# furiosa-ai/eta-inversion

Hardware: AMD Instinct MI355X
Metric: images/sec SD1.5 512^2 50-step etainv+ptp (higher is better)
Workload: dtype bf16; 1 GPU; etainv+ptp, SD1.5-shaped UNet (seeded synthetic weights), 512x512 (64x64 latents), 50 DDIM steps, 32 image pairs per GPU per step, eta [[0.6, 0], [1, 0.7]], n=10 noise candidates, cfg 7.5/1; images_per_gpu=32, unet_sample_forwards_per_image_reference=300

## Files before the change

### eta-inversion_amd/csrc/attention.hip

```cpp
#include <cstdlib>
#include <type_traits>

#include "common.h"
#include "kernels.h"
#include "self_attn_route.h"

namespace etainv {

template <typename T> struct Frag;
template <> struct Frag<f16> {
  typedef f16x8 v8;
  typedef f16x4 v4;
  static __device__ __forceinline__ f32x4 mfma(v8 a, v8 b, f32x4 c) { return __builtin_amdgcn_mfma_f32_16x16x32_f16(a, b, c, 0, 0, 0); }
};
template <> struct Frag<bf16> {
  typedef bf16x8 v8;
  typedef bf16x4 v4;
  static __device__ __forceinline__ f32x4 mfma(v8 a, v8 b, f32x4 c) { return __builtin_amdgcn_mfma_f32_16x16x32_bf16(a, b, c, 0, 0, 0); }
};

constexpr float NEG_BIG = -1.0e30f;

__device__ __forceinline__ void row_roles(int b, int n_img, int& half, int& role, int& img) {
  half = b / (2 * n_img);
// ... 657 lines not shown
        for (int qb = 0; qb < QB; ++qb) {
          v8 pf[4];
#pragma unroll
          for (int ks = 0; ks < 4; ++ks)
#pragma unroll
            for (int e = 0; e < 8; ++e) pf[ks][e] = (T)__builtin_amdgcn_exp2f(s[qb][ks >> 1][(ks & 1) * 8 + e]);
#pragma unroll
          for (int ks = 0; ks < 4; ++ks)
#pragma unroll
            for (int dt = 0; dt < DT; ++dt) o[qb][dt] = Frag32<T>::mfma(vf[ks][dt], pf[ks], o[qb][dt]);
        }
        if (j + 1 < ntiles) store_p(0, cur ^ 1);
        __syncthreads();
      }
    }

    const int q_base = qblk * QI + wid * (32 * QB);
#pragma unroll
    for (int qb = 0; qb < QB; ++qb) {
      const float l = __shfl(o[qb][GEO::LT][GEO::LI], r + 32 * GEO::LH, 64);
      const float inv = 1.f / l;
      const int query = q_base + qb * 32 + r;
      T* op = out + ((int64_t)b * N + query) * C + hd * D + 4 * h;
#pragma unroll
      for (int g4 = 0; g4 < D / 8; ++g4) {
        const int dt = g4 >> 2, i0 = (g4 & 3) * 4;
        T v[4] = {(T)(o[qb][dt][i0] * inv), (T)(o[qb][dt][i0 + 1] * inv), (T)(o[qb][dt][i0 + 2] * inv), (T)(o[qb][dt][i0 + 3] * inv)};
        *reinterpret_cast<u32x2*>(op + 8 * g4) = *reinterpret_cast<u32x2*>(v);
      }
    }
  }
}

template <typename T, int D, int QT, bool EDIT>
__global__ void __launch_bounds__(256) cross_attn_kernel(const T* __restrict__ q, const T* __restrict__ kv, T* __restrict__ out,
                                                         CrossParams p, int row0) {
  typedef typename Frag<T>::v8 v8;
  typedef typename Frag<T>::v4 v4;
  constexpr int DP = (D + 31) / 32 * 32;
  constexpr int KS = DP / 32;
  constexpr int DT = (D + 15) / 16;
  constexpr int NCH = D / 8;
  constexpr int KC = 96;
  constexpr int KT = 5;
  constexpr int KSTR = DP + 8;
  constexpr int VSTR = KC + 8;
  constexpr int PSTR = 81;

  extern __shared__ __attribute__((aligned(16))) char smem[];
  T* sK = reinterpret_cast<T*>(smem);
  T* sKs = sK + KC * KSTR;
  T* sVt = EDIT ? sKs + KC * KSTR : sKs;
  float* sP = reinterpret_cast<float*>(sVt + DT * 16 * VSTR);
  float* sTab = sP + 4 * QT * 16 * PSTR;

  const int tid = threadIdx.x, lane = tid & 63, wid = tid >> 6;
  const int fr = lane & 15, q4 = lane >> 4;
  int bx = blockIdx.x, gxn = gridDim.x, h = blockIdx.y, bz = blockIdx.z;
  if (p.xcd_gx > 0) {
    const int lin = blockIdx.x, xcd = lin & 7, t = lin >> 3;
    h = t % p.heads;
    const int c = (t / p.heads) * 8 + xcd;
    gxn = p.xcd_gx;
    bx = c % gxn;
    bz = c / gxn;
  }
// ... 18 lines not shown
  const bool do_edit = EDIT && p.edit && p.layout == 2 && is_cond && role == 1;
  const bool do_store = p.map_layer >= 0 && is_cond;
  const int bs = b - p.n_img;

  for (int idx = tid; idx < KC * (KSTR / 8); idx += 256) {
    const int key = idx / (KSTR / 8), ch = idx % (KSTR / 8);
    u32x4 a = {0u, 0u, 0u, 0u}, s = {0u, 0u, 0u, 0u};
    if (key < p.n_ctx && ch < NCH) {
      a = *reinterpret_cast<const u32x4*>(kv + ((int64_t)b * p.n_ctx + key) * C2 + h * D + ch * 8);
      if (do_edit) s = *reinterpret_cast<const u32x4*>(kv + ((int64_t)bs * p.n_ctx + key) * C2 + h * D + ch * 8);
    }
    *reinterpret_cast<u32x4*>(sK + key * KSTR + ch * 8) = a;
    if (EDIT) *reinterpret_cast<u32x4*>(sKs + key * KSTR + ch * 8) = s;
  }
  for (int idx = tid; idx < KC * NCH; idx += 256) {
    const int key = idx % KC, ch = idx / KC;
    u32x4 c = {0u, 0u, 0u, 0u};
    if (key < p.n_ctx) c = *reinterpret_cast<const u32x4*>(kv + ((int64_t)b * p.n_ctx + key) * C2 + C + h * D + ch * 8);
    const T* e = reinterpret_cast<const T*>(&c);
#pragma unroll
    for (int j = 0; j < 8; ++j) sVt[(ch * 8 + j) * VSTR + key] = e[j];
  }
  if (EDIT && do_edit && tid < p.n_ctx) {
    int mp = p.mapper ? p.mapper[img * 77 + tid] : 0;
    if (mp < 0) mp += p.n_ctx;
    sTab[0 * 80 + tid] = __builtin_bit_cast(float, mp);
    sTab[1 * 80 + tid] = p.alphas ? p.alphas[img * 77 + tid] : 0.f;
    sTab[2 * 80 + tid] = p.equalizer ? p.equalizer[img * 77 + tid] : 1.f;
    sTab[3 * 80 + tid] = p.cross_alpha[img * 77 + tid];
  }
  __syncthreads();

  constexpr bool QPF = D <= 80;
  u32x4 qn[QPF ? QT : 1][QPF ? 2 : 1][QPF ? KS : 1];
  auto load_q = [&](int qb, int qt, int brow, u32x4 (&dst)[QPF ? KS : 1]) __attribute__((always_inline)) {
    int query = qb * (64 * QT) + wid * (16 * QT) + qt * 16 + fr;
    query = query < N ? query : N - 1;
    const T* qp = q + ((int64_t)brow * N + query) * C + h * D;
#pragma unroll
    for (int ks = 0; ks < KS; ++ks) {
      const int d0 = ks * 32 + q4 * 8;
      u32x4 v = {0u, 0u, 0u, 0u};
      if (d0 < D) v = *reinterpret_cast<const u32x4*>(qp + d0);
      dst[ks] = v;
    }
  };
  auto load_block = [&](int qb) __attribute__((always_inline)) {
    if constexpr (QPF) {
#pragma unroll
      for (int qt = 0; qt < QT; ++qt) {
        load_q(qb, qt, b, qn[qt][0]);
        if (do_edit) load_q(qb, qt, bs, qn[qt][1]);
      }
    }
  };
  if (bx * (64 * QT) < N) load_block(bx);
  for (int qb = bx; qb * (64 * QT) < N; qb += gxn) {
  u32x4 qc[QPF ? QT : 1][QPF ? 2 : 1][QPF ? KS : 1];
  if constexpr (QPF) {
#pragma unroll
    for (int qt = 0; qt < QT; ++qt)
#pragma unroll
      for (int e = 0; e < 2; ++e)
#pragma unroll
        for (int ks = 0; ks < KS; ++ks) qc[qt][e][ks] = qn[qt][e][ks];
    if ((qb + gxn) * (64 * QT) < N) load_block(qb + gxn);
  }
#pragma unroll
  for (int qt = 0; qt < QT; ++qt) {
    const int q_base = qb * (64 * QT) + wid * (16 * QT);
    int query = q_base + qt * 16 + fr;
    const bool q_ok = query < N;
    query = q_ok ? query : N - 1;
    float* sPw = sP + ((wid * QT + qt) * 16 + fr) * PSTR;

    auto probs = [&](int brow, const T* keys, f32x4 (&pr)[KT]) {
      const T* qp = q + ((int64_t)brow * N + query) * C + h * D;
      f32x4 s[KT];
#pragma unroll
      for (int kt = 0; kt < KT; ++kt) s[kt] = (f32x4){0.f, 0.f, 0.f, 0.f};
#pragma unroll
      for (int ks = 0; ks < KS; ++ks) {
        const int d0 = ks * 32 + q4 * 8;
        u32x4 v = {0u, 0u, 0u, 0u};
        if constexpr (QPF) v = qc[qt][brow == b ? 0 : 1][ks];
        else if (d0 < D) v = *reinterpret_cast<const u32x4*>(qp + d0);
        v8 qf = *reinterpret_cast<v8*>(&v);
#pragma unroll
        for (int kt = 0; kt < KT; ++kt) {
          v8 kf = *reinterpret_cast<const v8*>(keys + (kt * 16 + fr) * KSTR + ks * 32 + q4 * 8);
          s[kt] = Frag<T>::mfma(kf, qf, s[kt]);
        }
      }
      float mx = NEG_BIG;
#pragma unroll
      for (int kt = 0; kt < KT; ++kt)
#pragma unroll
        for (int r = 0; r < 4; ++r) {
          float v = s[kt][r] * p.scale_log2;
          if (kt * 16 + q4 * 4 + r >= p.n_ctx) v = NEG_BIG;
          s[kt][r] = v;
          mx = fmaxf(mx, v);
        }
      mx = fmaxf(mx, __shfl_xor(mx, 16, 64));
      mx = fmaxf(mx, __shfl_xor(mx, 32, 64));
      float rs = 0.f;
#pragma unroll
      for (int kt = 0; kt < KT; ++kt)
#pragma unroll
        for (int r = 0; r < 4; ++r) {
          float e = __builtin_amdgcn_exp2f(s[kt][r] - mx);
          s[kt][r] = e;
          rs += e;
        }
      rs += __shfl_xor(rs, 16, 64);
      rs += __shfl_xor(rs, 32, 64);
      const float inv = 1.f / rs;
#pragma unroll
      for (int kt = 0; kt < KT; ++kt) pr[kt] = s[kt] * inv;
    };

    f32x4 pr[KT];
    if (do_edit) {
      f32x4 ps[KT];
      probs(bs, sKs, ps);
#pragma unroll
      for (int kt = 0; kt < KT; ++kt)
#pragma unroll
        for (int r = 0; r < 4; ++r) sPw[kt * 16 + q4 * 4 + r] = ps[kt][r];
      __builtin_amdgcn_fence(__ATOMIC_RELEASE, "workgroup");
      __builtin_amdgcn_wave_barrier();
      probs(b, sK, pr);
#pragma unroll
      for (int kt = 0; kt < KT; ++kt)
#pragma unroll
        for (int r = 0; r < 4; ++r) {
          const int key = kt * 16 + q4 * 4 + r;
          if (key < p.n_ctx) {
            const float tg = pr[kt][r];
            float rep;
            if (p.replace_mat) {
              const float* mrow = p.replace_mat + (int64_t)img * 77 * 77 + key;
              rep = 0.f;
              for (int w = 0; w < p.n_ctx; ++w) rep += sPw[w] * mrow[w * 77];
            } else {
              const int mp = __builtin_bit_cast(int, sTab[0 * 80 + key]);
              const float a = sTab[1 * 80 + key];
              rep = sPw[mp] * a + tg * (1.f - a);
            }
            rep *= sTab[2 * 80 + key];
            const float ca = sTab[3 * 80 + key];
            pr[kt][r] = rep * ca + (1.f - ca) * tg;
          }
        }
    } else {
      probs(b, sK, pr);
    }

    if (do_store && q_ok) {
      float* mp = p.maps_acc + (((((int64_t)p.map_layer * p.n_img_cap + img) * 2 + role) * p.heads + h) * N + query) * 77;
#pragma unroll
      for (int kt = 0; kt < KT; ++kt)
#pragma unroll
        for (int r = 0; r < 4; ++r) {
          const int key = kt * 16 + q4 * 4 + r;
          if (key < p.n_ctx) mp[key] += pr[kt][r];
        }
    }

    v8 pf[3];
#pragma unroll
    for (int kt = 0; kt < 6; ++kt)
#pragma unroll
      for (int r = 0; r < 4; ++r) pf[kt >> 1][(kt & 1) * 4 + r] = (kt < KT) ? (T)pr[kt < KT ? kt : 0][r] : (T)0.f;
    f32x4 acc[DT];
#pragma unroll
    for (int dt = 0; dt < DT; ++dt) acc[dt] = (f32x4){0.f, 0.f, 0.f, 0.f};
#pragma unroll
    for (int ks = 0; ks < 3; ++ks)
#pragma unroll
      for (int dt = 0; dt < DT; ++dt) {
        const T* vp = sVt + (dt * 16 + fr) * VSTR + ks * 32 + q4 * 4;
        v4 lo = *reinterpret_cast<const v4*>(vp);
        v4 hi = *reinterpret_cast<const v4*>(vp + 16);
        v8 vf = __builtin_shufflevector(lo, hi, 0, 1, 2, 3, 4, 5, 6, 7);
        acc[dt] = Frag<T>::mfma(vf, pf[ks], acc[dt]);
      }
    if (q_ok) {
      T* op = out + ((int64_t)b * N + query) * C + h * D;
#pragma unroll
      for (int dt = 0; dt < DT; ++dt) {
        const int dc = dt * 16 + q4 * 4;
        if (dc < D) {
          T o[4] = {(T)acc[dt][0], (T)acc[dt][1], (T)acc[dt][2], (T)acc[dt][3]};
          *reinterpret_cast<u32x2*>(op + dc) = *reinterpret_cast<u32x2*>(o);
        }
      }
    }
  }
  }
}

template <typename T, int D, int QB, int OCC>
static int launch_self40(const void* qkv, void* out, int b, int n, int heads, int mode, int n_img, int q_prescaled, hipStream_t s, int first_row = 0, int head_major = 0) {
  const int hm_rows = head_major ? b : 0;
  const int nqb = cdiv(n, 128 * QB);
  const bool remap = ((b * heads) % 8) == 0;
  const float q_scale = q_prescaled ? 1.0f : (1.0f / sqrtf((float)D)) * 1.4426950408889634f;
  constexpr size_t lds = A32<D>::LDS;
  ProfScope prof(PROF_SELF_ATTN, 4.0 * (double)b * heads * (double)n * (double)n * D, s);
  if constexpr (lds > 64 * 1024) {
    allow_dynamic_lds<&self_attn40_kernel<T, D, true, QB, OCC>>(lds);
    allow_dynamic_lds<&self_attn40_kernel<T, D, false, QB, OCC>>(lds);
  }
  if (remap)
    hipLaunchKernelGGL((self_attn40_kernel<T, D, true, QB, OCC>), dim3(nqb * heads * b), dim3(256), lds, s, (const T*)qkv, (T*)out, n, heads, q_scale, mode, n_img, nqb, first_row, hm_rows);
  else
    hipLaunchKernelGGL((self_attn40_kernel<T, D, false, QB, OCC>), dim3(nqb, heads, b), dim3(256), lds, s, (const T*)qkv, (T*)out, n, heads, q_scale, mode, n_img, nqb, first_row, hm_rows);
  ETAINV_LAUNCH_CHECK();
  return 0;
}

template <typename T, int D, int QB, int NW>
static int launch_self40q(const void* qkv, void* out, int b, int n, int heads, int mode, int n_img, int q_prescaled, hipStream_t s, int first_row, int head_major, int n_cu) {
  const int hm_rows = head_major ? b : 0;
  const int nqb = n / (32 * QB * NW);
  const int n_items = nqb * heads * b;
  const int remap = ((b * heads) % 8) == 0;
  const float q_scale = q_prescaled ? 1.0f : (1.0f / sqrtf((float)D)) * 1.4426950408889634f;
  constexpr size_t lds = (size_t)(4 * (A32<D>::KBUF + A32<D>::VBUF) + A32<D>::VBUF) * 2;
  allow_dynamic_lds<&self_attn40q_kernel<T, D, QB, NW, false>>(lds);
// ... 21 lines not shown
  }
  return n_cu[dev];
}

int launch_self_attention_mode(const void* qkv, void* out, int b, int n, int heads, int d, int mode, int n_img, int dtype,
                               hipStream_t s, int q_prescaled, int first_row, int head_major) {
  ETAINV_CHECK((!head_major && !q_prescaled) || self_attn_prescaled_hm_ok(d, dtype), "head-major QKV planes / pre-scaled queries: head_dim 40 / 80 on the 16-bit kernels only");
  ETAINV_CHECK(qkv && out && b > 0 && n > 0, "bad arguments");
  ETAINV_CHECK(mode >= 0 && mode <= 3, "self-attention mode: 0 plain, 1 ptp self-replace, 2 masactrl, 3 plug-and-play");
  ETAINV_CHECK(mode != 3 || (n_img > 0 && first_row == 0 && b == 3 * n_img), "plug-and-play mode needs the 3*n_img layout [u_s, u_t, c_t] x n_img with first_row == 0");
  ETAINV_CHECK(mode == 0 || mode == 3 || (n_img > 0 && ((first_row >= 0 && b + first_row == 4 * n_img && (first_row == 0 || (first_row == n_img && mode == 1))) ||
                                                        (first_row < 0 && b == 3 * n_img && mode == 1))),
               "ptp / masactrl modes need the 4*n_img backward layout (ptp: optionally without its first n_img rows, or rows [u_t, c_t, c_s] with first_row < 0)");
  if (dtype == ETAINV_F32) return launch_self_attention_f32(qkv, out, b, n, heads, d, mode, n_img, s, first_row);
  ETAINV_CHECK(d == 40 || d == 80 || d == 160, "head_dim must be 40, 80 or 160");
  const int n_cu = device_cu_count();
  const SelfAttnRoute route = self_attn_route(b, n, heads, d, n_cu, env_flag("ETAINV_A40_PERSIST", true), env_flag("ETAINV_A80_PERSIST", true));
  ETAINV_DISPATCH_HALF(dtype, T, switch (route) {
    case SELF_D40_ONE_BLOCK_PER_WAVE: return launch_self40<T, 40, 1, 2>(qkv, out, b, n, heads, mode, n_img, q_prescaled, s, first_row, head_major);
    case SELF_D40_PERSISTENT: return launch_self40q<T, 40, 4, 4>(qkv, out, b, n, heads, mode, n_img, q_prescaled, s, first_row, head_major, n_cu);
    case SELF_D40_TWO_BLOCK: return launch_self40<T, 40, 2, 2>(qkv, out, b, n, heads, mode, n_img, q_prescaled, s, first_row, head_major);
    case SELF_D80_PERSISTENT: return launch_self40q<T, 80, 2, 4>(qkv, out, b, n, heads, mode, n_img, q_prescaled, s, first_row, head_major, n_cu);
    case SELF_D80: return launch_self40<T, 80, 1, 2>(qkv, out, b, n, heads, mode, n_img, q_prescaled, s, first_row, head_major);
    case SELF_D160: return launch_self40<T, 160, 1, 1>(qkv, out, b, n, heads, mode, n_img, q_prescaled, s, first_row, head_major);
  });
  return 0;
}

template <typename T, int D>
static int launch_cross_t(const void* q, const void* kv, void* out, int b, const CrossParams& p, hipStream_t s) {
  constexpr int QT = 2;
  constexpr int DP = (D + 31) / 32 * 32, DT = (D + 15) / 16;
  const size_t lds_edit = (size_t)(2 * 96 * (DP + 8) + DT * 16 * (96 + 8)) * sizeof(T) + (size_t)(4 * QT * 16 * 81 + 4 * 80) * sizeof(float);
  const size_t lds_plain = (size_t)(96 * (DP + 8) + DT * 16 * (96 + 8)) * sizeof(T);
  allow_dynamic_lds<&cross_attn_kernel<T, D, QT, true>>(lds_edit);
  allow_dynamic_lds<&cross_attn_kernel<T, D, QT, false>>(lds_plain);
  ProfScope prof(PROF_CROSS_ATTN, 4.0 * (double)b * p.heads * (double)p.N * (double)p.n_ctx * D, s);
  const int nqb = cdiv(p.N, 64 * QT);
  auto launch = [&](bool edit, int row0, int rows) {
    static const int target_env = getenv("ETAINV_CROSS_BLOCKS") ? std::max(64, atoi(getenv("ETAINV_CROSS_BLOCKS"))) : 0;
    const int target = target_env ? target_env : p.N >= 2048 ? (edit ? 2048 : 6144) : 1024;
    const int cap = target_env ? nqb : p.N <= 256 ? 1 : p.N <= 1024 ? 2 : p.N <= 4096 ? 8 : nqb;
    const int gx = std::max(1, std::min(std::min(nqb, cap), cdiv(target, rows * p.heads)));
    const bool xcd_heads = env_flag("ETAINV_CROSS_XCD", true);
    CrossParams pl = p;
    dim3 grid(gx, p.heads, rows);
    if (xcd_heads && (gx * rows) % 8 == 0) {
      pl.xcd_gx = gx;
      grid = dim3(gx * p.heads * rows);
    }
    if (edit)
      hipLaunchKernelGGL((cross_attn_kernel<T, D, QT, true>), grid, dim3(256), lds_edit, s, (const T*)q, (const T*)kv, (T*)out, pl, row0);
    else
      hipLaunchKernelGGL((cross_attn_kernel<T, D, QT, false>), grid, dim3(256), lds_plain, s, (const T*)q, (const T*)kv, (T*)out, pl, row0);
  };
  if (p.edit && p.layout == 2) {
    const int edit0 = 3 * p.n_img - p.first_row;
    launch(false, 0, edit0);
    launch(true, edit0, b - edit0);
  } else {
    launch(false, 0, b);
  }
  ETAINV_LAUNCH_CHECK();
  return 0;
}

int launch_cross_attention_p(const void* q, const void* kv, void* out, int b, int d, const CrossParams& p, int dtype, hipStream_t s) {
// ... 22 lines not shown
```

### eta-inversion_amd/csrc/ppgemm.hip

```cpp
#include <cstdio>
#include <cstdlib>
#include <type_traits>
#include <vector>

#include "common.h"
#include "kernels.h"

namespace etainv {

namespace {

template <typename T> struct PMfma;
template <> struct PMfma<f16> {
  typedef f16x8 frag;
  static __device__ __forceinline__ f32x4 run(frag a, frag b, f32x4 c) { return __builtin_amdgcn_mfma_f32_16x16x32_f16(a, b, c, 0, 0, 0); }
};
template <> struct PMfma<bf16> {
  typedef bf16x8 frag;
  static __device__ __forceinline__ f32x4 run(frag a, frag b, f32x4 c) { return __builtin_amdgcn_mfma_f32_16x16x32_bf16(a, b, c, 0, 0, 0); }
};

#define PP_VMCNT(n) __builtin_amdgcn_s_waitcnt(0x0F70 | ((n) & 15) | (((n) >> 4) << 14))
#define PP_LGKMCNT0() __builtin_amdgcn_s_waitcnt(0xC07F)
#define PP_DMA(BYTES_INSN, voff32, sbase, ldsaddr) \
  asm volatile("s_mov_b32 m0, %2\n\ts_nop 0\n\t" BYTES_INSN " %0, %1" : : "v"(voff32), "s"(sbase), "s"(__builtin_amdgcn_readfirstlane(ldsaddr)) : "memory")

constexpr int PBM = 256, PBK = 64;
constexpr int PMT = 4;

__device__ __forceinline__ float dualn_row_sum16(float x) {
  x += __builtin_bit_cast(float, __builtin_amdgcn_update_dpp(0, __builtin_bit_cast(int, x), 0xB1, 0xf, 0xf, true));
  x += __builtin_bit_cast(float, __builtin_amdgcn_update_dpp(0, __builtin_bit_cast(int, x), 0x4E, 0xf, 0xf, true));
  x += __builtin_bit_cast(float, __builtin_amdgcn_update_dpp(0, __builtin_bit_cast(int, x), 0x141, 0xf, 0xf, true));
  x += __builtin_bit_cast(float, __builtin_amdgcn_update_dpp(0, __builtin_bit_cast(int, x), 0x140, 0xf, 0xf, true));
  return x;
}

template <int HN> struct DualN {
  static constexpr int NT = HN / 32;
  static constexpr int WN = HN / 2;
  static constexpr int BN2 = 2 * HN;
  static constexpr int PASSES = BN2 / 64;
  static constexpr int A_BYTES = PBM * PBK * 2, B_BYTES = BN2 * PBK * 2, SLOT = A_BYTES + B_BYTES;
  static constexpr int OFF_BIAS = 2 * SLOT, OFF_S = OFF_BIAS + 2 * BN2 * 4, OFF_STAT = OFF_S + 2 * BN2 * 4, LDS = OFF_STAT + 2 * PBM * 2 * 4;
};

template <typename T, int HN, int EPI, bool RES, int STAT, bool A2 = false>
__global__ void __launch_bounds__(512, 2) pp_dualn_kernel(IGemmParams p) {
  typedef typename PMfma<T>::frag frag;
  typedef DualN<HN> D;
  constexpr int NT = D::NT, WN = D::WN, BN2 = D::BN2, PASSES = D::PASSES;
  constexpr bool LNC = EPI != 0;
  static_assert((HN == 160 && EPI <= 2) || (HN == 128 && EPI == 3), "instantiations");
  static_assert(!LNC || (!RES && !STAT), "a LayerNorm consumer has no residual and emits no statistics");
  extern __shared__ __attribute__((aligned(16))) char smem[];
  float* sBias = reinterpret_cast<float*>(smem + D::OFF_BIAS);
  float* sS = reinterpret_cast<float*>(smem + D::OFF_S);
  float* sStat = reinterpret_cast<float*>(smem + D::OFF_STAT);

  const int tid = threadIdx.x, lane = tid & 63;
  const int wid = __builtin_amdgcn_readfirstlane(tid >> 6);
  const int wm = wid >> 1, wn = wid & 1;
  const int fr = lane & 15, fq = lane >> 4;
  const bool late = wid >= 4;

  const int K1 = p.c1, K = A2 ? p.c1 + p.c2 : p.c1, N = p.N;
  const int nk = K / PBK, nk1 = K1 / PBK;
  const int tiles_n = N / BN2;
  const int total_tiles = (p.M / PBM) * tiles_n;
  const int G = gridDim.x;
  const int my_tiles = (total_tiles - (int)blockIdx.x + G - 1) / G;
  if (my_tiles <= 0) return;
  auto tile_origin = [&](int i, int& m0, int& n0) __attribute__((always_inline)) {
    int v = blockIdx.x + i * G;
    if ((total_tiles & 7) == 0) v = (v & 7) * (total_tiles >> 3) + (v >> 3);
    const int tm = v / tiles_n;
    m0 = tm * PBM;
    n0 = (v - tm * tiles_n) * BN2;
  };
  const int total_steps = my_tiles * nk;
  const bool no_dma = p.debug & 1, no_epi = p.debug & 2, no_store = p.debug & 8, no_gelu = p.debug & 16;
  const bool fake_store = p.debug & 64;
  const bool has_bias = p.bias != nullptr;

  const unsigned lrow = tid >> 3;
  unsigned voff[PASSES];
#pragma unroll
  for (int q = 0; q < PASSES; ++q) voff[q] = ((lrow + 64 * q) * (unsigned)K + (((tid & 7) ^ (lrow & 7)) << 3)) * 2u;
  unsigned voa1[A2 ? 4 : 1], voa2[A2 ? 4 : 1];
  if constexpr (A2) {
#pragma unroll
    for (int q = 0; q < 4; ++q) {
      voa1[q] = ((lrow + 64 * q) * (unsigned)K1 + (((tid & 7) ^ (lrow & 7)) << 3)) * 2u;
      voa2[q] = ((lrow + 64 * q) * (unsigned)p.c2 + (((tid & 7) ^ (lrow & 7)) << 3)) * 2u;
    }
  }
  const int wrow_b = wid * 8 * PBK * 2;
  const unsigned lds0 = (unsigned)(unsigned long long)(__attribute__((address_space(3))) char*)smem;
  const char* a_base = nullptr;
  const char* a_base2 = nullptr;
  const char* w_base = nullptr;
  int a_tile = 0, a_kt = 0, a_cnt = 0;
  int b_tile = 0, b_kt = 0, b_cnt = 0;
  auto set_a = [&](int tile) __attribute__((always_inline)) {
    int m0, n0;
    tile_origin(tile, m0, n0);
    a_base = reinterpret_cast<const char*>(p.a1) + (int64_t)m0 * K1 * 2;
    if constexpr (A2) a_base2 = reinterpret_cast<const char*>(p.a2) + (int64_t)m0 * p.c2 * 2;
  };
  auto set_b = [&](int tile) __attribute__((always_inline)) {
    int m0, n0;
    tile_origin(tile, m0, n0);
    w_base = reinterpret_cast<const char*>(p.w) + (int64_t)n0 * K * 2;
    if (wid < BN2 / 64) {
      const unsigned db = ((tile & 1) * BN2 + wid * 64) * 4;
      if (has_bias) PP_DMA("global_load_lds_dword", (unsigned)(lane * 4), reinterpret_cast<const char*>(p.bias + n0 + wid * 64), lds0 + D::OFF_BIAS + db);
      if constexpr (LNC) PP_DMA("global_load_lds_dword", (unsigned)(lane * 4), reinterpret_cast<const char*>(p.ln_s + n0 + wid * 64), lds0 + D::OFF_S + db);
    }
    if constexpr (LNC)
      PP_DMA("global_load_lds_dword", (unsigned)(lane * 4), reinterpret_cast<const char*>(p.ln_stat + (int64_t)m0 * 2 + wid * 64),
             lds0 + D::OFF_STAT + ((tile & 1) * 512 + wid * 64) * 4);
  };
  auto issue_a = [&]() __attribute__((always_inline)) {
    if (!no_dma) {
      const unsigned d = lds0 + (a_cnt & 1) * D::SLOT + wrow_b;
      if constexpr (A2) {
        const bool second = a_kt >= nk1;
        const char* g = second ? a_base2 + (a_kt - nk1) * (PBK * 2) : a_base + a_kt * (PBK * 2);
        const unsigned v0 = second ? voa2[0] : voa1[0], v1 = second ? voa2[1] : voa1[1], v2 = second ? voa2[2] : voa1[2], v3 = second ? voa2[3] : voa1[3];
        PP_DMA("global_load_lds_dwordx4", v0, g, d);
        PP_DMA("global_load_lds_dwordx4", v1, g, d + 1 * (64 * PBK * 2));
        PP_DMA("global_load_lds_dwordx4", v2, g, d + 2 * (64 * PBK * 2));
        PP_DMA("global_load_lds_dwordx4", v3, g, d + 3 * (64 * PBK * 2));
      } else {
      const char* g = a_base + a_kt * (PBK * 2);
      PP_DMA("global_load_lds_dwordx4", voff[0], g, d);
      PP_DMA("global_load_lds_dwordx4", voff[1], g, d + 1 * (64 * PBK * 2));
      PP_DMA("global_load_lds_dwordx4", voff[2], g, d + 2 * (64 * PBK * 2));
      PP_DMA("global_load_lds_dwordx4", voff[3], g, d + 3 * (64 * PBK * 2));
      }
    }
    ++a_cnt;
    if (++a_kt == nk) {
      a_kt = 0;
      if (++a_tile < my_tiles) set_a(a_tile);
    }
  };
  auto issue_b = [&](auto q0_tag, auto q1_tag) __attribute__((always_inline)) {
    constexpr int q0 = decltype(q0_tag)::value, q1 = decltype(q1_tag)::value;
    if (!no_dma) {
      const char* g = w_base + b_kt * (PBK * 2);
      const unsigned d = lds0 + (b_cnt & 1) * D::SLOT + D::A_BYTES + wrow_b;
#pragma unroll
      for (int q = q0; q < q1; ++q) PP_DMA("global_load_lds_dwordx4", voff[q], g, d + q * (64 * PBK * 2));
    }
    if constexpr (q1 == PASSES) {
      ++b_cnt;
      if (++b_kt == nk) {
        b_kt = 0;
        if (++b_tile < my_tiles) set_b(b_tile);
      }
    }
  };

  f32x4 acc0[PMT][NT], acc1[PMT][NT];
#pragma unroll
  for (int i = 0; i < PMT; ++i)
#pragma unroll
    for (int j = 0; j < NT; ++j) acc0[i][j] = acc1[i][j] = (f32x4){0.f, 0.f, 0.f, 0.f};
  u32x4 fa[PMT] = {}, fb[NT] = {};
  unsigned a_rd[2], b_rd[2];
#pragma unroll
  for (int kk = 0; kk < 2; ++kk) {
    a_rd[kk] = ((wm * 64 + fr) * PBK + (((kk * 4 + fq) ^ (fr & 7)) << 3)) * 2;
    b_rd[kk] = D::A_BYTES + ((wn * WN + fr) * PBK + (((kk * 4 + fq) ^ (fr & 7)) << 3)) * 2;
  }
  auto read_a = [&](int slot, auto kk_tag) __attribute__((always_inline)) {
    const char* ba = smem + slot * D::SLOT + a_rd[decltype(kk_tag)::value];
#pragma unroll
    for (int i = 0; i < PMT; ++i) fa[i] = *reinterpret_cast<const u32x4*>(ba + i * (16 * PBK * 2));
  };
  auto read_b = [&](int slot, auto kk_tag, auto nh_tag) __attribute__((always_inline)) {
    const char* bb = smem + slot * D::SLOT + b_rd[decltype(kk_tag)::value] + decltype(nh_tag)::value * (HN * PBK * 2);
#pragma unroll
    for (int j = 0; j < NT; ++j) fb[j] = *reinterpret_cast<const u32x4*>(bb + j * (16 * PBK * 2));
  };
  auto cluster = [&](auto nh_tag) __attribute__((always_inline)) {
    constexpr int NH = decltype(nh_tag)::value;
    __builtin_amdgcn_sched_barrier(0);
    __builtin_amdgcn_s_setprio(1);
#pragma unroll
    for (int i = 0; i < PMT; ++i)
#pragma unroll
      for (int j = 0; j < NT; ++j) {
        if constexpr (NH == 0) acc0[i][j] = PMfma<T>::run(__builtin_bit_cast(frag, fb[j]), __builtin_bit_cast(frag, fa[i]), acc0[i][j]);
        else acc1[i][j] = PMfma<T>::run(__builtin_bit_cast(frag, fb[j]), __builtin_bit_cast(frag, fa[i]), acc1[i][j]);
      }
    __builtin_amdgcn_s_setprio(0);
    __builtin_amdgcn_sched_barrier(0);
  };

  T* const out = reinterpret_cast<T*>(p.out);
  const T* const res = reinterpret_cast<const T*>(p.residual);
  auto store_blocks = [&](T* prow, auto& po, auto nb_tag, int hm_d, int hm_skip) __attribute__((always_inline)) {
    constexpr int NB = decltype(nb_tag)::value;
    if (no_store) return;
    auto at = [&](int col) __attribute__((always_inline)) { return prow + col + (col >= hm_d ? hm_skip : 0); };
    if (fake_store) {
#pragma unroll
      for (int k = 0; k + 1 < NB; k += 2) {
        const u32x4 v = {po[k][0], po[k][1], po[k + 1][0], po[k + 1][1]};
        *reinterpret_cast<u32x4*>(prow + (k >> 1) * 512) = v;
      }
      if constexpr (NB & 1) *reinterpret_cast<u32x2*>(prow + (NB >> 1) * 512) = po[NB - 1];
      return;
    }
// ... 167 lines not shown
          }
          float mu = sum * (1.0f / (float)(NT * 4)), m2 = 0.f;
#pragma unroll
          for (int j = 0; j < NT; ++j) {
            T o[4];
            *reinterpret_cast<u32x2*>(o) = po[j];
#pragma unroll
            for (int q = 0; q < 4; ++q) { const float d = to_f32(o[q]) - mu; m2 += d * d; }
          }
          {
            const float mo = __shfl_xor(mu, 16, 64), qo = __shfl_xor(m2, 16, 64);
            const bool odd = fq & 1;
            float ma = odd ? mo : mu, mb = odd ? mu : mo, qa = odd ? qo : m2, qb = odd ? m2 : qo;
            float d = mb - ma;
            ma += 0.5f * d;
            qa += qb + d * d * (0.5f * (float)(NT * 4));
            const float mo2 = __shfl_xor(ma, 32, 64), qo2 = __shfl_xor(qa, 32, 64);
            const bool hi = fq >> 1;
            float m_lo = hi ? mo2 : ma, m_hi = hi ? ma : mo2, q_lo = hi ? qo2 : qa, q_hi = hi ? qa : qo2;
            d = m_hi - m_lo;
            mu = m_lo + 0.5f * d;
            m2 = q_lo;
            m2 += q_hi + d * d * (0.5f * (float)(2 * NT * 4));
          }
          if (fq == 0) *reinterpret_cast<f32x2*>(p.stat_out + ((int64_t)(mrow + i * 16) * p.stat_P + n0 / 80 + wn) * 2) = (f32x2){mu, m2};
        }
      }
    }
  };

  typedef std::integral_constant<int, 0> I0;
  typedef std::integral_constant<int, 1> I1;
  constexpr int QA = 2, QB = PASSES == 5 ? 4 : 3;
  set_a(0);
  set_b(0);
  issue_a();
  issue_b(I0{}, std::integral_constant<int, PASSES>{});
  if (total_steps > 1) { issue_a(); PP_VMCNT(4); } else { PP_VMCNT(0); }
  __builtin_amdgcn_s_barrier();
  if (late) __builtin_amdgcn_s_barrier();

  int ct_kt = 0, ct_tile = 0;
  for (int s = 0; s < total_steps; ++s) {
    const int slot = s & 1;
    const bool next = s + 1 < total_steps;
    if (s > 0 && ct_kt == 0 && !no_epi) {
      epilogue_half(I0{}, ct_tile - 1);
      epilogue_half(I1{}, ct_tile - 1);
    }
    const bool issue_w = next;
    if (issue_w) issue_b(I0{}, std::integral_constant<int, QA>{});
    read_a(slot, I0{});
    read_b(slot, I0{}, I0{});
    PP_LGKMCNT0();
    __builtin_amdgcn_sched_barrier(0);
    __builtin_amdgcn_s_barrier();
    cluster(I0{});
    __builtin_amdgcn_s_barrier();
    if (issue_w) issue_b(std::integral_constant<int, QA>{}, std::integral_constant<int, QB>{});
    read_b(slot, I0{}, I1{});
    PP_LGKMCNT0();
    __builtin_amdgcn_sched_barrier(0);
    __builtin_amdgcn_s_barrier();
    cluster(I1{});
    __builtin_amdgcn_s_barrier();
    if (issue_w) issue_b(std::integral_constant<int, QB>{}, std::integral_constant<int, PASSES>{});
    read_a(slot, I1{});
    read_b(slot, I1{}, I0{});
    PP_LGKMCNT0();
    __builtin_amdgcn_sched_barrier(0);
    __builtin_amdgcn_s_barrier();
    cluster(I0{});
    __builtin_amdgcn_s_barrier();
    PP_VMCNT(0);
    if (s + 2 < total_steps) issue_a();
    read_b(slot, I1{}, I1{});
    PP_LGKMCNT0();
    __builtin_amdgcn_sched_barrier(0);
    __builtin_amdgcn_s_barrier();
    cluster(I1{});
    __builtin_amdgcn_s_barrier();
    if (++ct_kt == nk) { ct_kt = 0; ++ct_tile; }
  }
  if (!no_epi) {
    epilogue_half(I0{}, ct_tile - 1);
    epilogue_half(I1{}, ct_tile - 1);
  }
  if (!late) __builtin_amdgcn_s_barrier();
}

}

static int dualn_kind(const IGemmParams& p, int dtype) {
  if (!env_flag("ETAINV_DUALN", true) || (dtype != ETAINV_F16 && dtype != ETAINV_BF16)) return -1;
  if (p.taps != 1 || p.rowvec || p.out_f32 || p.out_nchw || p.w_batch_stride || p.ksplit > 1) return -1;
  if (p.a2 && (p.geglu || p.ln_stat || p.residual || p.stat_out || p.hm_heads || p.c2 % PBK != 0 || p.c2 <= 0 || !env_flag("ETAINV_DUALN_A2", true))) return -1;
  if (p.stat_out && p.rows_per_batch % 64 != 0) return -1;
  if (p.M % PBM != 0 || p.c1 % PBK != 0 || p.c1 < 2 * PBK) return -1;
  int kind;
  if (p.geglu) {
    if (!p.ln_stat || !p.ln_s || !p.bias || p.residual || p.stat_out || p.hm_heads || p.N % 256 != 0) return -1;
    kind = 3;
  } else if (p.ln_stat) {
    if (!p.ln_s || !p.bias || p.residual || p.stat_out || p.N % 320 != 0) return -1;
    kind = p.hm_heads ? 2 : 1;
    if (kind == 2 && ((p.hm_dim != 40 && p.hm_dim != 80) || p.hm_heads != 8 || p.N != 3 * 8 * p.hm_dim || p.hm_tokens % 256 != 0 || p.M % p.hm_tokens != 0)) return -1;
  } else {
    if (p.hm_heads || p.N % 320 != 0) return -1;
    kind = 0;
  }
  static const int min_tiles = env_int("ETAINV_DUALN_MIN_TILES", 192);
  const int64_t tiles = (int64_t)(p.M / PBM) * (p.N / (kind == 3 ? 256 : 320));
  const int64_t rounds = (tiles + 255) / 256;
  if (tiles < min_tiles || tiles * 5 < rounds * 256 * 4) return -1;
  return kind;
}
bool pp_dualn_applicable(const IGemmParams& p, int dtype) { return dualn_kind(p, dtype) >= 0; }
bool pp_dualn_hm_ok(const IGemmParams& p, int dtype) { return dualn_kind(p, dtype) == 2; }

template <typename T, int HN, int EPI, bool RES, int STAT, bool A2 = false>
static void launch_dualn_t(const IGemmParams& p, int grid, hipStream_t s) {
  allow_dynamic_lds<&pp_dualn_kernel<T, HN, EPI, RES, STAT, A2>>(DualN<HN>::LDS);
  hipLaunchKernelGGL((pp_dualn_kernel<T, HN, EPI, RES, STAT, A2>), dim3(grid), dim3(512), DualN<HN>::LDS, s, p);
}

int launch_pp_dualn(const IGemmParams& p_in, int dtype, hipStream_t s, int* stat_P) {
  IGemmParams p = p_in;
  const int kind = dualn_kind(p, dtype);
  ETAINV_CHECK(kind >= 0, "not a dual-N launch (ask pp_dualn_applicable first)");
  if (p.stat_out) p.stat_P = p.stat_kind == 1 ? 64 : p.N / 80;
  if (stat_P) *stat_P = p.stat_out ? p.stat_P : 0;
  IGemmPlan& plan = igemm_last_plan();
  plan.bm = PBM;
  plan.bn = kind == 3 ? 256 : 320;
  plan.form = kind;
  const int tiles = (p.M / PBM) * (p.N / (kind == 3 ? 256 : 320));
  static const int grid_cap = std::max(1, env_int("ETAINV_DUALN_GRID", 256));
  const int grid = std::min(tiles, grid_cap);
  ETAINV_DISPATCH_HALF(dtype, T, {
    if (kind == 3) launch_dualn_t<T, 128, 3, false, 0>(p, grid, s);
    else if (kind == 2) launch_dualn_t<T, 160, 2, false, 0>(p, grid, s);
    else if (kind == 1) launch_dualn_t<T, 160, 1, false, 0>(p, grid, s);
    else if (p.residual) {
      if (p.stat_out && p.stat_kind == 1) launch_dualn_t<T, 160, 0, true, 2>(p, grid, s);
      else if (p.stat_out) launch_dualn_t<T, 160, 0, true, 1>(p, grid, s);
      else launch_dualn_t<T, 160, 0, true, 0>(p, grid, s);
    } else {
      if (p.stat_out && p.stat_kind == 1) launch_dualn_t<T, 160, 0, false, 2>(p, grid, s);
      else if (p.stat_out) launch_dualn_t<T, 160, 0, false, 1>(p, grid, s);
      else if (p.a2) launch_dualn_t<T, 160, 0, false, 0, true>(p, grid, s);
      else launch_dualn_t<T, 160, 0, false, 0>(p, grid, s);
    }
  });
  ETAINV_LAUNCH_CHECK();
  return 0;
}
// ... 3 lines not shown
```

Before: 5.928 images/s.

## Batch cross-attention query tiles, stage output through LDS, use permlane swaps

```diff
diff --git a/eta-inversion_amd/csrc/attention.hip b/eta-inversion_amd/csrc/attention.hip
--- a/eta-inversion_amd/csrc/attention.hip
+++ b/eta-inversion_amd/csrc/attention.hip
@@ -713,6 +713,32 @@
   }
 }
 
+template <bool SWAP> __device__ __forceinline__ float quad_max(float v) {
+  if constexpr (SWAP) {
+    float a = v, b = v;
+    asm volatile("s_nop 1\n\tv_permlane16_swap_b32 %0, %1" : "+v"(a), "+v"(b));
+    a = fmaxf(a, b);
+    b = a;
+    asm volatile("s_nop 1\n\tv_permlane32_swap_b32 %0, %1" : "+v"(a), "+v"(b));
+    return fmaxf(a, b);
+  } else {
+    v = fmaxf(v, __shfl_xor(v, 16, 64));
+    return fmaxf(v, __shfl_xor(v, 32, 64));
+  }
+}
+template <bool SWAP> __device__ __forceinline__ float quad_sum(float v) {
+  if constexpr (SWAP) {
+    float a = v, b = v;
+    asm volatile("s_nop 1\n\tv_permlane16_swap_b32 %0, %1" : "+v"(a), "+v"(b));
+    a = a + b;
+    b = a;
+    asm volatile("s_nop 1\n\tv_permlane32_swap_b32 %0, %1" : "+v"(a), "+v"(b));
+    return a + b;
+  } else {
+    v += __shfl_xor(v, 16, 64);
+    return v + __shfl_xor(v, 32, 64);
+  }
+}
 template <typename T, int D, int QT, bool EDIT>
 __global__ void __launch_bounds__(256) cross_attn_kernel(const T* __restrict__ q, const T* __restrict__ kv, T* __restrict__ out,
                                                          CrossParams p, int row0) {
@@ -797,6 +823,10 @@
   __syncthreads();
 
   constexpr bool QPF = D <= 80;
+  constexpr bool SWAP = D == 160;
+  constexpr bool WIDE_O = D <= 80 && !EDIT;
+  constexpr int OSTR = D + 8;
+  T* sOw = reinterpret_cast<T*>(sP) + wid * (QT * 16 * OSTR);
   u32x4 qn[QPF ? QT : 1][QPF ? 2 : 1][QPF ? KS : 1];
   auto load_q = [&](int qb, int qt, int brow, u32x4 (&dst)[QPF ? KS : 1]) __attribute__((always_inline)) {
     int query = qb * (64 * QT) + wid * (16 * QT) + qt * 16 + fr;
@@ -831,116 +861,141 @@
         for (int ks = 0; ks < KS; ++ks) qc[qt][e][ks] = qn[qt][e][ks];
     if ((qb + gxn) * (64 * QT) < N) load_block(qb + gxn);
   }
-#pragma unroll
-  for (int qt = 0; qt < QT; ++qt) {
+  {
     const int q_base = qb * (64 * QT) + wid * (16 * QT);
-    int query = q_base + qt * 16 + fr;
-    const bool q_ok = query < N;
-    query = q_ok ? query : N - 1;
-    float* sPw = sP + ((wid * QT + qt) * 16 + fr) * PSTR;
-
-    auto probs = [&](int brow, const T* keys, f32x4 (&pr)[KT]) {
-      const T* qp = q + ((int64_t)brow * N + query) * C + h * D;
-      f32x4 s[KT];
-#pragma unroll
-      for (int kt = 0; kt < KT; ++kt) s[kt] = (f32x4){0.f, 0.f, 0.f, 0.f};
+    int query[QT];
+    bool q_ok[QT];
+#pragma unroll
+    for (int g = 0; g < QT; ++g) {
+      query[g] = q_base + g * 16 + fr;
+      q_ok[g] = query[g] < N;
+      query[g] = q_ok[g] ? query[g] : N - 1;
+    }
+
+    auto probs = [&](int brow, const T* keys, f32x4 (&pr)[QT][KT]) {
+      f32x4 s[QT][KT];
+#pragma unroll
+      for (int g = 0; g < QT; ++g)
+#pragma unroll
+        for (int kt = 0; kt < KT; ++kt) s[g][kt] = (f32x4){0.f, 0.f, 0.f, 0.f};
 #pragma unroll
       for (int ks = 0; ks < KS; ++ks) {
         const int d0 = ks * 32 + q4 * 8;
-        u32x4 v = {0u, 0u, 0u, 0u};
-        if constexpr (QPF) v = qc[qt][brow == b ? 0 : 1][ks];
-        else if (d0 < D) v = *reinterpret_cast<const u32x4*>(qp + d0);
-        v8 qf = *reinterpret_cast<v8*>(&v);
+        v8 qf[QT];
+#pragma unroll
+        for (int g = 0; g < QT; ++g) {
+          u32x4 v = {0u, 0u, 0u, 0u};
+          if constexpr (QPF) v = qc[g][brow == b ? 0 : 1][ks];
+          else if (d0 < D) v = *reinterpret_cast<const u32x4*>(q + ((int64_t)brow * N + query[g]) * C + h * D + d0);
+          qf[g] = *reinterpret_cast<v8*>(&v);
+        }
 #pragma unroll
         for (int kt = 0; kt < KT; ++kt) {
           v8 kf = *reinterpret_cast<const v8*>(keys + (kt * 16 + fr) * KSTR + ks * 32 + q4 * 8);
-          s[kt] = Frag<T>::mfma(kf, qf, s[kt]);
-        }
-      }
-      float mx = NEG_BIG;
-#pragma unroll
-      for (int kt = 0; kt < KT; ++kt)
-#pragma unroll
-        for (int r = 0; r < 4; ++r) {
-          float v = s[kt][r] * p.scale_log2;
-          if (kt * 16 + q4 * 4 + r >= p.n_ctx) v = NEG_BIG;
-          s[kt][r] = v;
-          mx = fmaxf(mx, v);
-        }
-      mx = fmaxf(mx, __shfl_xor(mx, 16, 64));
-      mx = fmaxf(mx, __shfl_xor(mx, 32, 64));
-      float rs = 0.f;
-#pragma unroll
-      for (int kt = 0; kt < KT; ++kt)
-#pragma unroll
-        for (int r = 0; r < 4; ++r) {
-          float e = __builtin_amdgcn_exp2f(s[kt][r] - mx);
-          s[kt][r] = e;
-          rs += e;
-        }
-      rs += __shfl_xor(rs, 16, 64);
-      rs += __shfl_xor(rs, 32, 64);
-      const float inv = 1.f / rs;
-#pragma unroll
-      for (int kt = 0; kt < KT; ++kt) pr[kt] = s[kt] * inv;
+#pragma unroll
+          for (int g = 0; g < QT; ++g) s[g][kt] = Frag<T>::mfma(kf, qf[g], s[g][kt]);
+        }
+      }
+#pragma unroll
+      for (int g = 0; g < QT; ++g) {
+        float mx = NEG_BIG;
+#pragma unroll
+        for (int kt = 0; kt < KT; ++kt)
+#pragma unroll
+          for (int r = 0; r < 4; ++r) {
+            float v = s[g][kt][r] * p.scale_log2;
+            if (kt * 16 + q4 * 4 + r >= p.n_ctx) v = NEG_BIG;
+            s[g][kt][r] = v;
+            mx = fmaxf(mx, v);
+          }
+        mx = quad_max<SWAP>(mx);
+        float rs = 0.f;
+#pragma unroll
+        for (int kt = 0; kt < KT; ++kt)
+#pragma unroll
+          for (int r = 0; r < 4; ++r) {
+            float e = __builtin_amdgcn_exp2f(s[g][kt][r] - mx);
+            s[g][kt][r] = e;
+            rs += e;
+          }
+        rs = quad_sum<SWAP>(rs);
+        const float inv = 1.f / rs;
+#pragma unroll
+        for (int kt = 0; kt < KT; ++kt) pr[g][kt] = s[g][kt] * inv;
+      }
     };
 
-    f32x4 pr[KT];
+    f32x4 pr[QT][KT];
     if (do_edit) {
-      f32x4 ps[KT];
+      f32x4 ps[QT][KT];
       probs(bs, sKs, ps);
 #pragma unroll
-      for (int kt = 0; kt < KT; ++kt)
-#pragma unroll
-        for (int r = 0; r < 4; ++r) sPw[kt * 16 + q4 * 4 + r] = ps[kt][r];
+      for (int g = 0; g < QT; ++g) {
+        float* sPw = sP + ((wid * QT + g) * 16 + fr) * PSTR;
+#pragma unroll
+        for (int kt = 0; kt < KT; ++kt)
+#pragma unroll
+          for (int r = 0; r < 4; ++r) sPw[kt * 16 + q4 * 4 + r] = ps[g][kt][r];
+      }
       __builtin_amdgcn_fence(__ATOMIC_RELEASE, "workgroup");
       __builtin_amdgcn_wave_barrier();
       probs(b, sK, pr);
 #pragma unroll
-      for (int kt = 0; kt < KT; ++kt)
-#pragma unroll
-        for (int r = 0; r < 4; ++r) {
-          const int key = kt * 16 + q4 * 4 + r;
-          if (key < p.n_ctx) {
-            const float tg = pr[kt][r];
-            float rep;
-            if (p.replace_mat) {
-              const float* mrow = p.replace_mat + (int64_t)img * 77 * 77 + key;
-              rep = 0.f;
-              for (int w = 0; w < p.n_ctx; ++w) rep += sPw[w] * mrow[w * 77];
-            } else {
-              const int mp = __builtin_bit_cast(int, sTab[0 * 80 + key]);
-              const float a = sTab[1 * 80 + key];
-              rep = sPw[mp] * a + tg * (1.f - a);
+      for (int g = 0; g < QT; ++g) {
+        const float* sPw = sP + ((wid * QT + g) * 16 + fr) * PSTR;
+#pragma unroll
+        for (int kt = 0; kt < KT; ++kt)
+#pragma unroll
+          for (int r = 0; r < 4; ++r) {
+            const int key = kt * 16 + q4 * 4 + r;
+            if (key < p.n_ctx) {
+              const float tg = pr[g][kt][r];
+              float rep;
+              if (p.replace_mat) {
+                const float* mrow = p.replace_mat + (int64_t)img * 77 * 77 + key;
+                rep = 0.f;
+                for (int w = 0; w < p.n_ctx; ++w) rep += sPw[w] * mrow[w * 77];
+              } else {
+                const int mp = __builtin_bit_cast(int, sTab[0 * 80 + key]);
+                const float a = sTab[1 * 80 + key];
+                rep = sPw[mp] * a + tg * (1.f - a);
+              }
+              rep *= sTab[2 * 80 + key];
+              const float ca = sTab[3 * 80 + key];
+              pr[g][kt][r] = rep * ca + (1.f - ca) * tg;
             }
-            rep *= sTab[2 * 80 + key];
-            const float ca = sTab[3 * 80 + key];
-            pr[kt][r] = rep * ca + (1.f - ca) * tg;
           }
-        }
+      }
     } else {
       probs(b, sK, pr);
     }
 
-    if (do_store && q_ok) {
-      float* mp = p.maps_acc + (((((int64_t)p.map_layer * p.n_img_cap + img) * 2 + role) * p.heads + h) * N + query) * 77;
-#pragma unroll
-      for (int kt = 0; kt < KT; ++kt)
-#pragma unroll
-        for (int r = 0; r < 4; ++r) {
-          const int key = kt * 16 + q4 * 4 + r;
-          if (key < p.n_ctx) mp[key] += pr[kt][r];
-        }
-    }
-
-    v8 pf[3];
-#pragma unroll
-    for (int kt = 0; kt < 6; ++kt)
-#pragma unroll
-      for (int r = 0; r < 4; ++r) pf[kt >> 1][(kt & 1) * 4 + r] = (kt < KT) ? (T)pr[kt < KT ? kt : 0][r] : (T)0.f;
-    f32x4 acc[DT];
-#pragma unroll
-    for (int dt = 0; dt < DT; ++dt) acc[dt] = (f32x4){0.f, 0.f, 0.f, 0.f};
+    if (do_store) {
+#pragma unroll
+      for (int g = 0; g < QT; ++g)
+        if (q_ok[g]) {
+          float* mp = p.maps_acc + (((((int64_t)p.map_layer * p.n_img_cap + img) * 2 + role) * p.heads + h) * N + query[g]) * 77;
+#pragma unroll
+          for (int kt = 0; kt < KT; ++kt)
+#pragma unroll
+            for (int r = 0; r < 4; ++r) {
+              const int key = kt * 16 + q4 * 4 + r;
+              if (key < p.n_ctx) mp[key] += pr[g][kt][r];
+            }
+        }
+    }
+
+    v8 pf[QT][3];
+    f32x4 acc[QT][DT];
+#pragma unroll
+    for (int g = 0; g < QT; ++g) {
+#pragma unroll
+      for (int kt = 0; kt < 6; ++kt)
+#pragma unroll
+        for (int r = 0; r < 4; ++r) pf[g][kt >> 1][(kt & 1) * 4 + r] = (kt < KT) ? (T)pr[g][kt < KT ? kt : 0][r] : (T)0.f;
+#pragma unroll
+      for (int dt = 0; dt < DT; ++dt) acc[g][dt] = (f32x4){0.f, 0.f, 0.f, 0.f};
+    }
 #pragma unroll
     for (int ks = 0; ks < 3; ++ks)
 #pragma unroll
@@ -949,19 +1004,45 @@
         v4 lo = *reinterpret_cast<const v4*>(vp);
         v4 hi = *reinterpret_cast<const v4*>(vp + 16);
         v8 vf = __builtin_shufflevector(lo, hi, 0, 1, 2, 3, 4, 5, 6, 7);
-        acc[dt] = Frag<T>::mfma(vf, pf[ks], acc[dt]);
-      }
-    if (q_ok) {
-      T* op = out + ((int64_t)b * N + query) * C + h * D;
-#pragma unroll
-      for (int dt = 0; dt < DT; ++dt) {
-        const int dc = dt * 16 + q4 * 4;
-        if (dc < D) {
-          T o[4] = {(T)acc[dt][0], (T)acc[dt][1], (T)acc[dt][2], (T)acc[dt][3]};
-          *reinterpret_cast<u32x2*>(op + dc) = *reinterpret_cast<u32x2*>(o);
-        }
-      }
-    }
+#pragma unroll
+        for (int g = 0; g < QT; ++g) acc[g][dt] = Frag<T>::mfma(vf, pf[g][ks], acc[g][dt]);
+      }
+    if constexpr (WIDE_O) {
+#pragma unroll
+      for (int g = 0; g < QT; ++g)
+#pragma unroll
+        for (int dt = 0; dt < DT; ++dt) {
+          const int dc = dt * 16 + q4 * 4;
+          if (dc < D) {
+            T o[4] = {(T)acc[g][dt][0], (T)acc[g][dt][1], (T)acc[g][dt][2], (T)acc[g][dt][3]};
+            *reinterpret_cast<u32x2*>(sOw + ((g) * 16 + fr) * OSTR + dc) = *reinterpret_cast<u32x2*>(o);
+          }
+        }
+      __builtin_amdgcn_fence(__ATOMIC_RELEASE, "workgroup");
+      __builtin_amdgcn_wave_barrier();
+#pragma unroll
+      for (int i = 0; i < (QT * 16 * NCH + 63) / 64; ++i) {
+        const int c = lane + 64 * i;
+        const int tok = c / NCH, qy = q_base + tok;
+        if (c < QT * 16 * NCH && qy < N)
+          *reinterpret_cast<u32x4*>(out + ((int64_t)b * N + qy) * C + h * D + (c % NCH) * 8) = *reinterpret_cast<const u32x4*>(sOw + tok * OSTR + (c % NCH) * 8);
+      }
+      __builtin_amdgcn_fence(__ATOMIC_RELEASE, "workgroup");
+      __builtin_amdgcn_wave_barrier();
+    } else
+#pragma unroll
+    for (int g = 0; g < QT; ++g)
+      if (q_ok[g]) {
+        T* op = out + ((int64_t)b * N + query[g]) * C + h * D;
+#pragma unroll
+        for (int dt = 0; dt < DT; ++dt) {
+          const int dc = dt * 16 + q4 * 4;
+          if (dc < D) {
+            T o[4] = {(T)acc[g][dt][0], (T)acc[g][dt][1], (T)acc[g][dt][2], (T)acc[g][dt][3]};
+            *reinterpret_cast<u32x2*>(op + dc) = *reinterpret_cast<u32x2*>(o);
+          }
+        }
+      }
   }
   }
 }
@@ -1049,7 +1130,7 @@
   constexpr int QT = 2;
   constexpr int DP = (D + 31) / 32 * 32, DT = (D + 15) / 16;
   const size_t lds_edit = (size_t)(2 * 96 * (DP + 8) + DT * 16 * (96 + 8)) * sizeof(T) + (size_t)(4 * QT * 16 * 81 + 4 * 80) * sizeof(float);
-  const size_t lds_plain = (size_t)(96 * (DP + 8) + DT * 16 * (96 + 8)) * sizeof(T);
+  const size_t lds_plain = (size_t)(96 * (DP + 8) + DT * 16 * (96 + 8)) * sizeof(T) + (D <= 80 ? (size_t)4 * QT * 16 * (D + 8) * sizeof(T) : 0);
   allow_dynamic_lds<&cross_attn_kernel<T, D, QT, true>>(lds_edit);
   allow_dynamic_lds<&cross_attn_kernel<T, D, QT, false>>(lds_plain);
   ProfScope prof(PROF_CROSS_ATTN, 4.0 * (double)b * p.heads * (double)p.N * (double)p.n_ctx * D, s);
```

After: 5.943 images/s (median of 6 runs). Within noise of the previous version (+0.2%).

## Add triple-buffered LDS ring for the dual-N A2 GEMM path

Applied to the files above, without the earlier changes.

```diff
diff --git a/eta-inversion_amd/csrc/ppgemm.hip b/eta-inversion_amd/csrc/ppgemm.hip
--- a/eta-inversion_amd/csrc/ppgemm.hip
+++ b/eta-inversion_amd/csrc/ppgemm.hip
@@ -36,27 +36,39 @@
   return x;
 }
 
-template <int HN> struct DualN {
+#ifndef ETAINV_DUALN_RING3
+#define ETAINV_DUALN_RING3 1
+#endif
+constexpr bool dualn_ring3(int hn, int epi, bool a2) { return ETAINV_DUALN_RING3 && hn == 160 && epi == 0 && a2; }
+
+template <int HN, bool RING3> struct DualN {
   static constexpr int NT = HN / 32;
   static constexpr int WN = HN / 2;
   static constexpr int BN2 = 2 * HN;
   static constexpr int PASSES = BN2 / 64;
   static constexpr int A_BYTES = PBM * PBK * 2, B_BYTES = BN2 * PBK * 2, SLOT = A_BYTES + B_BYTES;
-  static constexpr int OFF_BIAS = 2 * SLOT, OFF_S = OFF_BIAS + 2 * BN2 * 4, OFF_STAT = OFF_S + 2 * BN2 * 4, LDS = OFF_STAT + 2 * PBM * 2 * 4;
+  static constexpr int UNIT = HN * PBK * 2;
+  static constexpr int OFF_B = 3 * A_BYTES;
+  static constexpr int OFF_BIAS = RING3 ? OFF_B + 3 * UNIT : 2 * SLOT;
+  static constexpr int OFF_S = OFF_BIAS + 2 * BN2 * 4, OFF_STAT = OFF_S + 2 * BN2 * 4;
+  static constexpr int LDS = RING3 ? OFF_S : OFF_STAT + 2 * PBM * 2 * 4;
+  static_assert(LDS <= 160 * 1024, "LDS of a CU");
 };
 
 template <typename T, int HN, int EPI, bool RES, int STAT, bool A2 = false>
 __global__ void __launch_bounds__(512, 2) pp_dualn_kernel(IGemmParams p) {
   typedef typename PMfma<T>::frag frag;
-  typedef DualN<HN> D;
+  constexpr bool RING3 = dualn_ring3(HN, EPI, A2);
+  typedef DualN<HN, RING3> D;
   constexpr int NT = D::NT, WN = D::WN, BN2 = D::BN2, PASSES = D::PASSES;
   constexpr bool LNC = EPI != 0;
   static_assert((HN == 160 && EPI <= 2) || (HN == 128 && EPI == 3), "instantiations");
   static_assert(!LNC || (!RES && !STAT), "a LayerNorm consumer has no residual and emits no statistics");
+  static_assert(!RING3 || D::LDS == 162304, "3 x 32 KB + 3 x 20 KB + the bias ring");
   extern __shared__ __attribute__((aligned(16))) char smem[];
   float* sBias = reinterpret_cast<float*>(smem + D::OFF_BIAS);
-  float* sS = reinterpret_cast<float*>(smem + D::OFF_S);
-  float* sStat = reinterpret_cast<float*>(smem + D::OFF_STAT);
+  float* sS = reinterpret_cast<float*>(smem + (LNC ? D::OFF_S : D::OFF_BIAS));
+  float* sStat = reinterpret_cast<float*>(smem + (LNC ? D::OFF_STAT : D::OFF_BIAS));
 
   const int tid = threadIdx.x, lane = tid & 63;
   const int wid = __builtin_amdgcn_readfirstlane(tid >> 6);
@@ -112,6 +124,13 @@
     int m0, n0;
     tile_origin(tile, m0, n0);
     w_base = reinterpret_cast<const char*>(p.w) + (int64_t)n0 * K * 2;
+    if constexpr (RING3) {
+      if (has_bias) {
+        const unsigned db = lds0 + D::OFF_BIAS + ((tile & 1) * BN2 + wid * 64) * 4;
+        PP_DMA("global_load_lds_dword", (unsigned)(lane * 4), reinterpret_cast<const char*>(p.bias + n0 + wid * 64), db);
+        if (wid == 0) PP_DMA("global_load_lds_dword", (unsigned)(lane * 4), reinterpret_cast<const char*>(p.bias + n0 + 256), db + 256 * 4);
+      }
+    } else
     if (wid < BN2 / 64) {
       const unsigned db = ((tile & 1) * BN2 + wid * 64) * 4;
       if (has_bias) PP_DMA("global_load_lds_dword", (unsigned)(lane * 4), reinterpret_cast<const char*>(p.bias + n0 + wid * 64), lds0 + D::OFF_BIAS + db);
@@ -162,6 +181,44 @@
       }
     }
   };
+  const unsigned grow = (wid & 3) * 8 + (lane >> 3);
+  const unsigned gchunk = (((lane & 7) ^ (lane >> 3)) << 3);
+  const unsigned vow = (grow * (unsigned)K + gchunk) * 2u, voa = (grow * (unsigned)K1 + gchunk) * 2u;
+  const unsigned voa_2 = A2 ? (grow * (unsigned)p.c2 + gchunk) * 2u : 0u;
+  const unsigned grow_b = (wid & 3) * 8 * PBK * 2;
+  auto ring_issue_a = [&](int slot) __attribute__((always_inline)) {
+    if (!no_dma) {
+      const unsigned d = lds0 + slot * D::A_BYTES + grow_b;
+      const char* g = a_base + a_kt * (PBK * 2);
+      unsigned v = voa;
+      int pass = 32 * K1 * 2;
+      if constexpr (A2) {
+        if (a_kt >= nk1) { g = a_base2 + (a_kt - nk1) * (PBK * 2); v = voa_2; pass = 32 * p.c2 * 2; }
+      }
+#pragma unroll
+      for (int q = 0; q < 8; ++q) PP_DMA("global_load_lds_dwordx4", v, g + (int64_t)q * pass, d + q * (32 * PBK * 2));
+    }
+    if (++a_kt == nk) {
+      a_kt = 0;
+      if (++a_tile < my_tiles) set_a(a_tile);
+    }
+  };
+  auto ring_issue_w = [&](auto h_tag, int slot, auto q0_tag, auto q1_tag) __attribute__((always_inline)) {
+    constexpr int h = decltype(h_tag)::value, q0 = decltype(q0_tag)::value, q1 = decltype(q1_tag)::value;
+    if (!no_dma) {
+      const char* g = w_base + b_kt * (PBK * 2) + (int64_t)h * HN * K * 2;
+      const unsigned d = lds0 + D::OFF_B + slot * D::UNIT + grow_b;
+      const int pass = 32 * K * 2;
+#pragma unroll
+      for (int q = q0; q < q1; ++q) PP_DMA("global_load_lds_dwordx4", vow, g + (int64_t)q * pass, d + q * (32 * PBK * 2));
+    }
+    if constexpr (h == 1 && q1 == 5) {
+      if (++b_kt == nk) {
+        b_kt = 0;
+        if (++b_tile < my_tiles) set_b(b_tile);
+      }
+    }
+  };
 
   f32x4 acc0[PMT][NT], acc1[PMT][NT];
 #pragma unroll
@@ -182,6 +239,16 @@
   };
   auto read_b = [&](int slot, auto kk_tag, auto nh_tag) __attribute__((always_inline)) {
     const char* bb = smem + slot * D::SLOT + b_rd[decltype(kk_tag)::value] + decltype(nh_tag)::value * (HN * PBK * 2);
+#pragma unroll
+    for (int j = 0; j < NT; ++j) fb[j] = *reinterpret_cast<const u32x4*>(bb + j * (16 * PBK * 2));
+  };
+  auto ring_read_a = [&](int slot, auto kk_tag) __attribute__((always_inline)) {
+    const char* ba = smem + slot * D::A_BYTES + a_rd[decltype(kk_tag)::value];
+#pragma unroll
+    for (int i = 0; i < PMT; ++i) fa[i] = *reinterpret_cast<const u32x4*>(ba + i * (16 * PBK * 2));
+  };
+  auto ring_read_b = [&](int unit, auto kk_tag) __attribute__((always_inline)) {
+    const char* bb = smem + (D::OFF_B - D::A_BYTES) + unit * D::UNIT + b_rd[decltype(kk_tag)::value];
 #pragma unroll
     for (int j = 0; j < NT; ++j) fb[j] = *reinterpret_cast<const u32x4*>(bb + j * (16 * PBK * 2));
   };
@@ -415,6 +482,74 @@
   typedef std::integral_constant<int, 0> I0;
   typedef std::integral_constant<int, 1> I1;
   constexpr int QA = 2, QB = PASSES == 5 ? 4 : 3;
+  int ct_kt = 0, ct_tile = 0;
+  if constexpr (RING3) {
+    typedef std::integral_constant<int, 2> I2;
+    typedef std::integral_constant<int, 4> I4;
+    typedef std::integral_constant<int, 5> I5;
+    if (!late) {
+      set_b(0);
+      ring_issue_w(I0{}, 0, I0{}, I5{});
+      ring_issue_w(I1{}, 1, I0{}, I5{});
+      PP_VMCNT(5);
+    } else {
+      set_a(0);
+      ring_issue_a(0);
+      if (total_steps > 1) ring_issue_a(1);
+      if (total_steps > 2) { ring_issue_a(2); PP_VMCNT(16); } else if (total_steps > 1) { PP_VMCNT(8); } else { PP_VMCNT(0); }
+    }
+    __builtin_amdgcn_s_barrier();
+    if (late) __builtin_amdgcn_s_barrier();
+    int ra = 0, u0 = 0, u1 = 1;
+    for (int s = 0; s < total_steps; ++s) {
+      const bool next = s + 1 < total_steps;
+      const int uf = 3 - u0 - u1;
+      if (s > 0 && ct_kt == 0 && !no_epi) {
+        epilogue_half(I0{}, ct_tile - 1);
+        epilogue_half(I1{}, ct_tile - 1);
+      }
+      const bool issue_w = !late && next;
+      if (issue_w) ring_issue_w(I0{}, uf, I0{}, I2{});
+      ring_read_a(ra, I0{});
+      ring_read_b(u0, I0{});
+      PP_LGKMCNT0();
+      __builtin_amdgcn_sched_barrier(0);
+      __builtin_amdgcn_s_barrier();
+      cluster(I0{});
+      if (!late) { if (next) PP_VMCNT(2); else PP_VMCNT(0); }
+      __builtin_amdgcn_s_barrier();
+      if (issue_w) ring_issue_w(I0{}, uf, I2{}, I4{});
+      ring_read_b(u1, I0{});
+      PP_LGKMCNT0();
+      __builtin_amdgcn_sched_barrier(0);
+      __builtin_amdgcn_s_barrier();
+      cluster(I1{});
+      __builtin_amdgcn_s_barrier();
+      if (issue_w) ring_issue_w(I0{}, uf, I4{}, I5{});
+      ring_read_a(ra, I1{});
+      ring_read_b(u0, I1{});
+      PP_LGKMCNT0();
+      __builtin_amdgcn_sched_barrier(0);
+      __builtin_amdgcn_s_barrier();
+      cluster(I0{});
+      __builtin_amdgcn_s_barrier();
+      if (!late) {
+        if (next) { ring_issue_w(I1{}, u0, I0{}, I5{}); PP_VMCNT(5); }
+      } else {
+        if (s + 3 < total_steps) { ring_issue_a(ra); PP_VMCNT(16); } else if (s + 2 < total_steps) { PP_VMCNT(8); } else { PP_VMCNT(0); }
+      }
+      ring_read_b(u1, I1{});
+      PP_LGKMCNT0();
+      __builtin_amdgcn_sched_barrier(0);
+      __builtin_amdgcn_s_barrier();
+      cluster(I1{});
+      __builtin_amdgcn_s_barrier();
+      if (++ct_kt == nk) { ct_kt = 0; ++ct_tile; }
+      ra = ra == 2 ? 0 : ra + 1;
+      u1 = u0;
+      u0 = uf;
+    }
+  } else {
   set_a(0);
   set_b(0);
   issue_a();
@@ -423,7 +558,6 @@
   __builtin_amdgcn_s_barrier();
   if (late) __builtin_amdgcn_s_barrier();
 
-  int ct_kt = 0, ct_tile = 0;
   for (int s = 0; s < total_steps; ++s) {
     const int slot = s & 1;
     const bool next = s + 1 < total_steps;
@@ -464,6 +598,7 @@
     cluster(I1{});
     __builtin_amdgcn_s_barrier();
     if (++ct_kt == nk) { ct_kt = 0; ++ct_tile; }
+  }
   }
   if (!no_epi) {
     epilogue_half(I0{}, ct_tile - 1);
@@ -503,8 +638,9 @@
 
 template <typename T, int HN, int EPI, bool RES, int STAT, bool A2 = false>
 static void launch_dualn_t(const IGemmParams& p, int grid, hipStream_t s) {
-  allow_dynamic_lds<&pp_dualn_kernel<T, HN, EPI, RES, STAT, A2>>(DualN<HN>::LDS);
-  hipLaunchKernelGGL((pp_dualn_kernel<T, HN, EPI, RES, STAT, A2>), dim3(grid), dim3(512), DualN<HN>::LDS, s, p);
+  constexpr int lds = DualN<HN, dualn_ring3(HN, EPI, A2)>::LDS;
+  allow_dynamic_lds<&pp_dualn_kernel<T, HN, EPI, RES, STAT, A2>>(lds);
+  hipLaunchKernelGGL((pp_dualn_kernel<T, HN, EPI, RES, STAT, A2>), dim3(grid), dim3(512), lds, s, p);
 }
 
 int launch_pp_dualn(const IGemmParams& p_in, int dtype, hipStream_t s, int* stat_P) {
```

Measured after the change: 5.809 images/s before, 5.810 images/s after, median of 3. No clear change (+0.0%).
